# JokerJohn/DCReg

Hardware: AMD Instinct MI355X
Metric: ICP iterations/sec (higher is better)
Workload: dtype f64

## Files before the change

dcreg_amd/csrc/device/context.hip:

```cpp
#include <algorithm>
#include <cmath>
#include <cstdarg>
#include <cstdio>
#include <cstdlib>
#include <chrono>
#include <cstring>
#include <string>
#include <vector>

#include <hip/hip_runtime.h>
#include <rocprim/device/device_radix_sort.hpp>
#include <rocprim/device/device_scan.hpp>

#include "../../../include/dcreg_debug.h"
#include "context.hpp"
#include "kernels.hpp"

namespace dcreg {

constexpr double kCountScale = 67108864.0;
constexpr size_t kSearchCountBytes = 64 * kCounterStride * sizeof(uint32_t);
static inline unsigned blocks_for(int64_t n, int bs) { return (unsigned)((n + bs - 1) / bs); }
static void drop_warm(dcreg_ctx *c);

// ... 1433 lines not shown
        }
        if (!L.p || search_bound_sq(c, L.p->search_radius) != ps.radius_sq_f) { c->fail("the pair targets were built for another search radius"); return DCREG_E_INVALID; }
    }
    L.n = c->n_src;
    if (L.frame_ids) {
        if (!L.state_ids || L.dbg || gated) { c->fail("frame launches are batched product launches"); return DCREG_E_INVALID; }
        L.n = 0;
        for (int i = 0; i < L.n_poses; ++i) {
            const int32_t f = L.frame_ids[i];
            if (f < 0 || (size_t)f >= L.fs->slice.size() || L.fs->slice[(size_t)f].y == 0u) { c->fail("frame %d is not loaded or empty", f); return DCREG_E_INVALID; }
            L.n = std::max<int64_t>(L.n, L.fs->slice[(size_t)f].y);
        }
    } else
    if (c->n_src <= 0) { c->fail("measure cloud is not set"); return DCREG_E_STATE; }
    L.kind = L.grid_ids ? LinKind::pairs : L.frame_ids ? LinKind::frames : gated ? LinKind::gated : (L.n_poses > 1 || L.state_ids) ? LinKind::batch :
             !L.dbg ? LinKind::single : stamps_only ? LinKind::stamps : LinKind::dump;
    if (!L.p && !gated && (c->roi_active || roi_wanted(c))) { c->fail("null argument"); return DCREG_E_INVALID; }
    const dcreg_lin_params *p = L.p;
    if (!p || !(p->search_radius > 0.0)) { c->fail("invalid linearisation parameters"); return DCREG_E_INVALID; }
    if (p->k != 5 && p->k != 0) { c->fail("only k = 5 is supported (icp_test_runner.cpp:1722)"); return DCREG_E_INVALID; }
    if (p->parameterization != DCREG_PARAM_SO3 && p->parameterization != DCREG_PARAM_EULER && p->parameterization != DCREG_PARAM_EULER_EXACT) { c->fail("unknown parameterization"); return DCREG_E_INVALID; }
    if (L.state_ids && c->opt_warm) {
        const int64_t n_states = L.frame_ids ? L.fs->n_states : c->n_batch_states;
        std::vector<uint8_t> seen((size_t)std::max<int64_t>(n_states, 1), 0);
        for (int i = 0; i < L.n_poses; ++i) {
            const int32_t sid = L.state_ids[i];
            if (sid < 0) continue;
            if ((int64_t)sid >= n_states) { c->fail("warm state %d was not reserved (dcreg_reserve_warm_states: %lld)", sid, (long long)n_states); return DCREG_E_INVALID; }
            if (seen[(size_t)sid]) { c->fail("warm state %d is used by two poses of one launch", sid); return DCREG_E_INVALID; }
            seen[(size_t)sid] = 1;
        }
    }
    return DCREG_OK;
}

static bool order_wanted(const dcreg_ctx *c, const LinLaunch &L) {
    return c->opt_dispatch_order && L.own() && c->n_groups >= 2 && blocks_for(L.n, kLinBlock) > 4u * (uint32_t)c->n_cus &&
           c->hint_misalign > 0.5 * c->map.grid.h;
}

static LinPlan lin_plan(const dcreg_ctx *c, const LinLaunch &L, bool fresh) {
    LinPlan P;
    P.kind = L.kind; P.n_poses = L.n_poses; P.nbx = blocks_for(L.n, kLinBlock);
    P.n_chunks = (P.nbx + kChunk - 1) / kChunk;
    const bool fused = L.n_poses == 1 || P.n_chunks == 1;
    P.direct = fused && L.n_poses == 1 && P.nbx <= (uint32_t)kChunk && c->opt_one_wave < 2;
    P.n_rows = P.direct ? (size_t)P.nbx : (fused ? (size_t)P.n_chunks * (size_t)P.n_poses : (size_t)P.n_poses);
    const bool dbg = L.kind == LinKind::dump || L.kind == LinKind::stamps;
    P.use_cert = L.kind != LinKind::dump && c->opt_use_cert;
    P.ordered = order_wanted(c, L) && c->order_valid && c->order_uneven;
    const bool known = c->last_searched >= 0 && c->last_points == L.n;
    const double f = known ? (double)c->last_searched / (double)L.n : -1.0;
    if ((L.kind == LinKind::single || L.kind == LinKind::gated) && c->opt_warm && !fresh && P.use_cert && L.a.count_scale != 0.0) {
        constexpr double kAdvanceLo = 0.005, kAdvanceHi = 0.70;
        const bool adv = c->opt_advance >= 2 || (c->opt_advance == 1 && P.nbx >= (uint32_t)c->opt_advance_min_blocks && known && f >= kAdvanceLo && f <= kAdvanceHi);
        constexpr double kTeamPassMaxPoints = 16384.0, kTeamPassMinFrac = 0.5, kTeamPassMinCellPts = 3.0;
        const double per_cell = (double)c->map.n / (double)std::max<uint32_t>(c->map.occupied, 1u);
        const bool team = c->opt_team_pass >= 2 || (c->opt_team_pass == 1 && L.n <= (int64_t)kTeamPassMaxPoints && known && f >= kTeamPassMinFrac &&
                                                    per_cell >= kTeamPassMinCellPts);
        P.pass = team ? LinPass::team : adv ? LinPass::advance : LinPass::none;
    }
    bool one_wave = false;
    if (L.n_poses > 1)
        one_wave = fused && !dbg && (c->opt_one_wave >= 2 || (c->opt_one_wave_batches && (uint64_t)L.n_poses * P.nbx >= (uint64_t)c->opt_one_wave_min_blocks));
    else if (!P.direct && !dbg && P.pass != LinPass::team) {
        const bool most = !L.uses_state(c) || fresh || !P.use_cert || (known && (double)c->last_searched >= c->opt_one_wave_min_frac * (double)L.n);
        one_wave = c->opt_one_wave >= 2 || (c->opt_one_wave == 1 && P.nbx >= (uint32_t)c->opt_one_wave_min_blocks && P.pass != LinPass::advance && most &&
                                            c->hint_misalign > c->opt_one_wave_min_cells * c->map.grid.h);
    }
    P.gate_inside = L.kind == LinKind::gated && c->opt_gate_in_kernel && P.nbx <= (uint32_t)kChunk && P.pass != LinPass::advance;
    P.body = (P.gate_inside && P.pass != LinPass::team) ? LinBody::gated : L.kind == LinKind::stamps ? LinBody::stamps : L.kind == LinKind::dump ? LinBody::dump :
             one_wave ? LinBody::one_wave : fused ? LinBody::fused : LinBody::chunked;
    P.pass_rows = P.pass == LinPass::advance && c->opt_advance_fused != 0 && !P.direct && P.body == LinBody::fused;
    return P;
}

static int stage_poses(dcreg_ctx *c, LinSlot &S, LinLaunch &L) {
    const int64_t n_states = L.frame_ids ? L.fs->n_states : c->n_batch_states;
    std::vector<uint8_t> &state_valid = L.frame_ids ? L.fs->state_valid : c->batch_state_valid;
    dcreg_ctx::StateKey &states_key = L.frame_ids ? L.fs->key : c->batch_state_key;
    const bool use_states = L.state_ids && c->opt_warm && n_states > 0;
    if (use_states && !(L.key == states_key)) {
        std::fill(state_valid.begin(), state_valid.end(), (uint8_t)0);
        states_key = L.key;
    }
    const int n_poses = L.n_poses;
    const size_t bytes = (size_t)n_poses * sizeof(PoseArg) + (L.frame_ids ? (size_t)n_poses * sizeof(uint2) : 0) +
                         (L.grid_ids ? (size_t)n_poses * sizeof(uint32_t) : 0);
    if (bytes > S.d_poses.cap()) {
        S.h_poses.reset(); S.d_poses.reset();
        const size_t cap = std::max<size_t>(bytes, 256 * (sizeof(PoseArg) + sizeof(uint2) + sizeof(uint32_t)));
        HIP_TRY(c, S.h_poses.alloc(cap, hipHostMallocDefault));
        if (S.d_poses.alloc(cap) != hipSuccess) { c->fail("hipMalloc(%zu B) failed", cap); return DCREG_E_NOMEM; }
    }
    PoseArg *hp = (PoseArg *)S.h_poses.data();
    for (int i = 0; i < n_poses; ++i) {
        std::memcpy(hp[i].R, L.R9 + 9 * i, sizeof(hp[i].R)); std::memcpy(hp[i].t, L.t3 + 3 * i, sizeof(hp[i].t));
        const bool has = use_states && L.state_ids[i] >= 0;
        hp[i].state = has ? (uint32_t)L.state_ids[i] : kNoIdx;
        hp[i].fresh = (has && state_valid[(size_t)L.state_ids[i]] != 0) ? 0u : 1u;
        if (has) state_valid[(size_t)L.state_ids[i]] = 1;
    }
    if (L.frame_ids) {
        uint2 *hs = (uint2 *)(S.h_poses.data() + (size_t)n_poses * sizeof(PoseArg));
        for (int i = 0; i < n_poses; ++i) hs[i] = L.fs->slice[(size_t)L.frame_ids[i]];
        L.d_slices = (const uint2 *)(S.d_poses.data() + (size_t)n_poses * sizeof(PoseArg));
    }
// ... 48 lines not shown
        if (c->d_adv_counts.ensure(c, (size_t)kCounterStride * P.nbx)) return DCREG_E_NOMEM;
        if (c->d_adv_counts.cap() != had || c->adv_counts_dirty) {
            HIP_TRY(c, hipMemsetAsync(c->d_adv_counts.data(), 0, sizeof(uint32_t) * c->d_adv_counts.cap(), c->stream));
            c->adv_counts_dirty = false;
        }
        L.a.adv_counts = c->d_adv_counts.data();
    }
    if (P.pass == LinPass::team && c->opt_team_stamps) {
        const uint32_t n_tiles = blocks_for(L.n, kTeamTile);
        if (c->d_team_stamps.ensure(c, (size_t)8 * (n_tiles + 1))) return DCREG_E_NOMEM;
        HIP_TRY(c, hipMemsetAsync(c->d_team_stamps.data(), 0, sizeof(unsigned long long) * 8 * (n_tiles + 1), c->stream));
        c->team_stamps_n = n_tiles;
    }
    free_tmp(S);
    if (L.dbg) {
        const dcreg_lin_debug *dbg = L.dbg; const size_t n = (size_t)L.n; DebugDev &dd = L.dd;
        bool oom = false;
        auto alloc = [&](size_t bytes, int fill) -> void * {
            DevBuf<unsigned char> b;
            if (b.alloc(bytes) != hipSuccess) { oom = true; return nullptr; }
            (void)hipMemsetAsync(b.data(), fill, bytes, c->stream);
            S.tmp_dev.push_back(std::move(b));
            return S.tmp_dev.back().data();
        };
        if (dbg->nn_idx) dd.nn_idx = (int32_t *)alloc(sizeof(int32_t) * 5 * n, 0xFF);
        if (dbg->nn_d2) dd.nn_d2 = (float *)alloc(sizeof(float) * 5 * n, 0);
        if (dbg->flag) dd.flag = (uint8_t *)alloc(n, 0);
        if (dbg->normal) dd.normal = (double *)alloc(sizeof(double) * 3 * n, 0);
        if (dbg->r) dd.r = (double *)alloc(sizeof(double) * n, 0);
        if (dbg->s) dd.s = (double *)alloc(sizeof(double) * n, 0);
        if (dbg->stats) dd.stats = (uint32_t *)alloc(sizeof(uint32_t) * n, 0);
        if (dbg->stamps) dd.stamps = (unsigned long long *)alloc(sizeof(unsigned long long) * 8 * (kLinBlock / 64) * (size_t)P.nbx, 0);
        if (oom) { free_tmp(S); drop_warm(c); c->fail("hipMalloc of the debug dump buffers failed"); return DCREG_E_NOMEM; }
    }
    L.a.use_cert = P.use_cert ? 1 : 0;
    L.a.search_count = c->opt_count_searches ? c->d_search_count.data() : nullptr;
    L.a.group_blocks = std::max<uint32_t>(c->group_blocks, 1u); L.a.n_groups = P.ordered ? c->n_groups : 0u;
    std::memcpy(L.a.group_order, c->group_order, sizeof(L.a.group_order));
    return DCREG_OK;
}

using LinKernel = decltype(&k_lin<0, true, true>);
template <bool FAST, bool SLICE = false, bool GRIDS = false>
static LinKernel lin_kernel(const LinPlan &P) {
    if constexpr (!SLICE) {
        if (P.kind == LinKind::pairs) return lin_kernel<FAST, true, true>(P);
        if (P.kind == LinKind::frames) return lin_kernel<FAST, true>(P);
        if (P.body == LinBody::gated) return k_lin<0, true, FAST, true>;
        if (P.body == LinBody::stamps) return k_lin<2, true, FAST>;
        if (P.body == LinBody::dump) return k_lin<1, true, FAST>;
    }
    if (P.one_wave()) return k_lin<0, true, FAST, false, true, SLICE, GRIDS>;
    return P.fused() ? k_lin<0, true, FAST, false, false, SLICE, GRIDS> : k_lin<0, false, FAST, false, false, SLICE, GRIDS>;
}

template <bool FAST>
static int lin_queue(dcreg_ctx *c, LinSlot &S, LinLaunch &L, const LinPlan &P) {
    const bool gated = L.kind == LinKind::gated, team = P.pass == LinPass::team, slice = L.kind == LinKind::frames || L.kind == LinKind::pairs;
    const uint32_t n = (uint32_t)L.n;
    const unsigned long long seq = ++c->seq;
    FinArgs fin{S.d_tickets.data(), S.h_out.dev(), seq, P.direct ? 1u : 0u, P.n_chunks};
    if (P.fused()) S.tickets_dirty = true;
    bool timed = c->opt_time_kernels > 0 && (c->launch_counter++ % (uint64_t)c->opt_time_kernels) == 0;
    if (timed && !S.ev0) timed = false;
    const uint32_t *abort_flag = nullptr;
    auto bail = [&](const char *what, hipError_t e) {
        if (e == hipSuccess) return DCREG_OK;
        free_tmp(S);
        if (gated) gate_call_off(c);
        drop_warm(c);
        c->fail("%s failed: %s", what, hipGetErrorString(e));
        return DCREG_E_DEVICE;
    };
    auto record = [&](hipEvent_t ev) { return bail("hipEventRecord", timed ? hipEventRecord(ev, c->stream) : hipSuccess); };
    GateArgs gt{nullptr, nullptr, 0ull, nullptr, nullptr, 0u};
    const PoseArg *lin_poses = L.d_poses;
    if (gated) {
        const unsigned long long want = ++c->gate_seq;
        if (P.gate_inside) {
            gt = GateArgs{c->h_gate.dev(), c->d_gate_dev.data(), want, team ? c->d_gate_pose.data() : nullptr, team ? c->d_gate_abort.data() : nullptr, L.one.fresh};
            if (team) abort_flag = c->d_gate_abort.data();
            else lin_poses = nullptr;
        } else {
            hipLaunchKernelGGL(k_gate, dim3(1), dim3(64), 0, c->stream, c->h_gate.dev(), want, c->d_gate_pose.data(), L.one.fresh, c->d_gate_abort.data());
            abort_flag = c->d_gate_abort.data();
        }
    }
    if (int rc = record(S.ev0)) return rc;
    if (P.pass == LinPass::advance) {
        const auto pass = P.pass_rows ? k_advance<FAST, true> : k_advance<FAST, false>;
        hipLaunchKernelGGL(pass, dim3(blocks_for(L.n, kAdvTile)), dim3(kLinBlock), 0, c->stream, c->d_src.data(), n, c->map.grid, L.one, L.d_poses, L.a,
                           P.pass_rows ? nullptr : c->d_adv_counts.data(), abort_flag, S.d_partials.data(), P.nbx, fin);
    }
    if (team) {
        const auto pass = P.gate_inside ? k_advance_team<FAST, true> : k_advance_team<FAST>;
        hipLaunchKernelGGL(pass, dim3(blocks_for(L.n, kTeamTile)), dim3(kWave), 0, c->stream, c->d_src.data(), n, c->map.grid, L.one, P.gate_inside ? nullptr : L.d_poses,
                           L.a, c->d_adv_counts.data(), P.gate_inside ? nullptr : abort_flag, c->opt_team_stamps ? c->d_team_stamps.data() : nullptr, gt);
    }
    if (P.pass != LinPass::none) {
        if (int rc = bail(team ? "team advance pass launch" : "advance pass launch", hipGetLastError())) return rc;
        c->n_advance_launches += 1;
    }
    const bool one = P.one_wave(); const auto lin = lin_kernel<FAST>(P);
    if (!P.pass_rows)
    hipLaunchKernelGGL(lin, dim3(one ? P.nbx * (kLinBlock / kWave) : P.nbx, (unsigned)P.n_poses), dim3(one ? kWave : kLinBlock), 0, c->stream,
                       slice ? L.fs->src.data() : c->d_src.data(), n, c->map.grid, L.one, lin_poses, L.a, S.d_partials.data(), P.nbx, fin, L.dd, abort_flag, gt,
                       L.d_slices, L.kind == LinKind::pairs ? c->pairs.d_grids.data() : nullptr, L.d_grid_ids);
    if (one)
        hipLaunchKernelGGL(slice ? k_sum_tiles<true> : k_sum_tiles<false>, dim3(P.n_chunks, (unsigned)P.n_poses), dim3(kLinBlock), 0, c->stream, S.d_partials.data(),
                           P.nbx, S.h_out.dev(), seq, abort_flag, L.d_slices);
    if (int rc = bail("linearisation kernel launch", hipGetLastError())) return rc;
    if (!P.fused()) {
        hipLaunchKernelGGL(slice ? k_finalize<true> : k_finalize<false>, dim3((unsigned)P.n_poses), dim3(kLinBlock), 0, c->stream, S.d_partials.data(), P.nbx,
                           S.h_out.dev(), seq, L.d_slices);
        if (int rc = bail("k_finalize launch", hipGetLastError())) return rc;
    }
    if (int rc = record(S.ev1)) return rc;
    if (const dcreg_lin_debug *dbg = L.dbg) {
        const DebugDev &dd = L.dd;
        hipError_t ce = hipSuccess;
        auto back = [&](void *dst, const void *srcp, size_t bytes) { if (ce == hipSuccess && srcp) ce = hipMemcpyAsync(dst, srcp, bytes, hipMemcpyDeviceToHost, c->stream); };
        back(dbg->nn_idx, dd.nn_idx, sizeof(int32_t) * 5 * n);
        back(dbg->nn_d2, dd.nn_d2, sizeof(float) * 5 * n);
        back(dbg->flag, dd.flag, (size_t)n);
        back(dbg->normal, dd.normal, sizeof(double) * 3 * n);
        back(dbg->r, dd.r, sizeof(double) * n);
        back(dbg->s, dd.s, sizeof(double) * n);
        back(dbg->stats, dd.stats, sizeof(uint32_t) * n);
        back(dbg->stamps, dd.stamps, sizeof(unsigned long long) * 8 * (kLinBlock / 64) * (size_t)P.nbx);
        if (ce != hipSuccess) { (void)hipStreamSynchronize(c->stream); return bail("copying the debug dump back", ce); }
    }
    c->n_launches += 1; c->n_poses_launched += P.n_poses; c->n_points_launched += (int64_t)P.n_poses * L.n;
    if (L.uses_state(c)) c->state_valid = true;
    S.pending = true; S.plan = P; S.timed = timed; S.seq = seq; S.sync = L.dbg != nullptr;
    S.coded = L.a.count_scale != 0.0;
    if (gated) {
        c->gate_slot = L.slot;
        c->gate_uses_state = L.uses_state(c); c->gate_state_was_valid = L.state_was_valid;
    }
    return DCREG_OK;
}

static int linearize_begin(dcreg_ctx *c, int slot, int n_poses, const double *R9, const double *t3, const int32_t *state_ids,
                           const dcreg_lin_params *p, dcreg_lin_debug *dbg_host, bool gated = false, const int32_t *frame_ids = nullptr,
                           const int32_t *grid_ids = nullptr) {
// ... 286 lines not shown

int dcreg_set_stream(dcreg_ctx *c, void *s) {
    if (!c) return DCREG_E_INVALID;
    if (int rc = refuse_in_flight(c)) return rc;
    (void)hipStreamSynchronize(c->stream);
    c->stream = s ? (hipStream_t)s : c->own_stream;
    return DCREG_OK;
}

int dcreg_set_option(dcreg_ctx *c, const char *key, double v) {
    if (!c || !key) return DCREG_E_INVALID;
    const std::string k(key);
    if (k == "cell") c->opt_cell = v;
    else if (k == "cell_factor") c->opt_cell_factor = v > 0.1 ? v : 2.0;
    else if (k == "use_certificates") c->opt_use_cert = v != 0.0;
    else if (k == "count_searches") {
        if (v != 0.0 && !c->d_search_count) {
            HIP_TRY(c, c->d_search_count.alloc(kSearchCountBytes / sizeof(unsigned long long)));
            HIP_TRY(c, hipMemsetAsync(c->d_search_count.data(), 0, kSearchCountBytes, c->stream));
        }
        c->opt_count_searches = v != 0.0;
    }
    else if (k == "cert_margin" || k == "cert_inflate" || k == "warm_start" || k == "fast_plane_fit") {
        if (c->gate_slot >= 0) { c->fail("a gated linearisation is queued: open or abort it before changing \"%s\"", key); return DCREG_E_STATE; }
        if (k == "cert_margin") c->opt_cert_margin = v >= 1e-4 ? std::min(v, 1.0) : 1e-4;
        else if (k == "cert_inflate") c->opt_cert_inflate = v >= 0.0 ? std::min(v, 1.0) : 0.0;
        else if (k == "warm_start") c->opt_warm = v != 0.0;
        else c->opt_fast_plane = v != 0.0;
        drop_warm(c);
    }
    else if (k == "wait_seconds") c->opt_wait_seconds = v > 0.0 ? v : 30.0;
    else if (k == "x_subdiv") { int sx = 1; while (sx < 16 && (double)(sx * 2) <= v) sx *= 2; c->opt_x_subdiv = sx; }
    else if (k == "time_kernels") { c->opt_time_kernels = v > 0.0 ? (int)v : 0; c->launch_counter = 0; }
    else if (k == "record_launches") { c->opt_record_launches = v != 0.0; if (v == 0.0) c->launch_series.clear(); }
    else if (k == "curve_x_scale") c->opt_curve_x_scale = (v > 0.0 && v <= 1.0) ? v : 1.0;
    else if (k == "roi_index") { c->opt_roi_index = (int)std::min(std::max(v, 0.0), 2.0); c->roi_built = false; }
    else if (k == "roi_margin") { c->opt_roi_margin = std::min(std::max(v, 0.0), 1.0e6); c->roi_built = false; }
    else if (k == "pair_max_table_entries") c->opt_pair_max_table_entries = (int64_t)std::min(std::max(v, 4096.0), 2147483648.0);
    else if (k == "pairs_max_bytes") c->opt_pairs_max_bytes = std::max(v, 0.0);
    else if (k == "visibility_max_bytes") c->opt_visibility_max_bytes = std::max(v, 0.0);
    else if (k == "visibility_order") c->opt_visibility_order = (int)v;
    else if (k == "max_table_entries") c->opt_max_table_entries = (int64_t)std::min(std::max(v, 1048576.0), 2147483648.0);
    else if (k == "advance") c->opt_advance = (int)v;
    else if (k == "advance_fused") c->opt_advance_fused = (int)v;
    else if (k == "one_wave") c->opt_one_wave = (int)v;
    else if (k == "one_wave_batches") c->opt_one_wave_batches = v != 0.0;
    else if (k == "one_wave_min_frac") c->opt_one_wave_min_frac = v;
    else if (k == "one_wave_min_cells") c->opt_one_wave_min_cells = v;
    else if (k == "one_wave_min_blocks") c->opt_one_wave_min_blocks = (int)v;
    else if (k == "gate_in_kernel") c->opt_gate_in_kernel = v != 0.0;
    else if (k == "team_stamps") c->opt_team_stamps = v != 0.0;
    else if (k == "team_pass") c->opt_team_pass = (int)v;
    else if (k == "advance_min_blocks") c->opt_advance_min_blocks = (int)v;
    else if (k == "team_search") c->opt_team_max = (int)v;
    else if (k == "spin") c->opt_spin = v != 0.0;
    else if (k == "far_bound") c->opt_far_bound = v != 0.0;
    else if (k == "dispatch_order") { c->opt_dispatch_order = v != 0.0; c->order_valid = false; }
    else if (k == "keep_source_order") c->opt_keep_source_order = v != 0.0;
    else if (k == "gap_field") c->opt_gap_field = v != 0.0;
    else if (k == "map_update") c->opt_map_update = v != 0.0 ? 1 : 0;
    else if (k == "normals_follow") c->opt_normals_follow = v != 0.0 ? 1 : 0;
    else if (k == "normals_follow_full_share") c->opt_normals_follow_full_share = std::min(std::max(v, 0.0), 1.0);
    else if (k == "gicp_epsilon") {
        if (!(v >= 1.0e-6 && v <= 1.0)) { c->fail("gicp_epsilon is %g: 1e-6 .. 1 expected", v); return DCREG_E_INVALID; }
        c->opt_gicp_epsilon = v;
    }
    else if (k == "robust_kernel") {
        if (!(v == (double)DCREG_ROBUST_NONE || v == (double)DCREG_ROBUST_HUBER || v == (double)DCREG_ROBUST_CAUCHY || v == (double)DCREG_ROBUST_GEMAN_MCCLURE)) {
            c->fail("robust_kernel is %g: 0 (none), 1 (Huber), 2 (Cauchy) or 3 (Geman-McClure) expected", v); return DCREG_E_INVALID;
        }
        c->opt_robust_kernel = (int)v;
    }
    else if (k == "robust_scale" || k == "gicp_robust_scale") {
        if (!(v >= 1.0e-6 && v <= 1.0e6)) { c->fail("%s is %g: 1e-6 .. 1e6 expected", key, v); return DCREG_E_INVALID; }
        (k == "robust_scale" ? c->opt_robust_scale : c->opt_gicp_robust_scale) = v;
    }
    else if (k == "voxels_source_cov") {
        if (!(v == 0.0 || v == 1.0)) { c->fail("voxels_source_cov is %g: 0 or 1 expected", v); return DCREG_E_INVALID; }
        c->opt_voxels_source_cov = (int)v;
    }
    else if (k == "map_grow_margin") c->opt_map_grow_margin = std::min(std::max(v, 0.0), 1.0e4);
    else { c->fail("unknown option '%s'", key); return DCREG_E_INVALID; }
    return DCREG_OK;
}

int dcreg_set_target(dcreg_ctx *c, const float *xyz, int64_t n, int64_t stride, double r) { return set_target(c, xyz, n, stride, r, false); }
int dcreg_set_target_device(dcreg_ctx *c, const float *xyz, int64_t n, int64_t stride, double r) { return set_target(c, xyz, n, stride, r, true); }
int dcreg_target_insert(dcreg_ctx *c, const float *xyz, int64_t n, int64_t stride, const double R[9], const double t[3], double min_spacing,
                        dcreg_map_update *info) {
    return map_insert(c, xyz, n, stride, false, false, R, t, min_spacing, info);
}
int dcreg_target_insert_device(dcreg_ctx *c, const float *d_xyz, int64_t n, int64_t stride, const double R[9], const double t[3], double min_spacing,
                               dcreg_map_update *info) {
    return map_insert(c, d_xyz, n, stride, true, false, R, t, min_spacing, info);
}
int dcreg_target_insert_source(dcreg_ctx *c, const double R[9], const double t[3], double min_spacing, dcreg_map_update *info) {
    return map_insert(c, nullptr, 0, 3, false, true, R, t, min_spacing, info);
}
int dcreg_target_crop(dcreg_ctx *c, const double lo[3], const double hi[3], dcreg_map_update *info) { return map_crop(c, lo, hi, info); }
int dcreg_target_get(const dcreg_ctx *c, float *xyz_out, int64_t capacity_points) { return target_get(c, xyz_out, capacity_points); }
int dcreg_debug_index_check(dcreg_ctx *c, int64_t mismatches[5]) {
    if (!c || !mismatches) return DCREG_E_INVALID;
    if (int rc = refuse_in_flight(c)) return rc;
    if (whole_map(c).n <= 0) { c->fail("no target"); return DCREG_E_STATE; }
    HIP_TRY(c, hipSetDevice(c->device));
    return index_check(c, mismatches);
// ... 431 lines not shown
```

dcreg_amd/csrc/device/context.hpp:

```cpp
#pragma once
#include <hip/hip_runtime.h>

#include <algorithm>
#include <chrono>
#include <cmath>
#include <cstdint>
#include <cstring>
#include <functional>
#include <utility>
#include <vector>

#include "../../../include/dcreg.h"
#include "kernels.hpp"

struct dcreg_lin_params;
struct dcreg_lin_out;
struct dcreg_lin_debug;

#define HIP_TRY(ctx, expr)                                                                       \
    do {                                                                                         \
        hipError_t e__ = (expr);                                                                 \
        if (e__ != hipSuccess) {                                                                 \
            (ctx)->fail("%s failed: %s (%s:%d)", #expr, hipGetErrorString(e__), __FILE__, __LINE__); \
            return DCREG_E_DEVICE;                                                               \
// ... 399 lines not shown
    double opt_one_wave_min_cells = 1.5;
    int opt_one_wave_min_blocks = 1024;
    unsigned long long gate_seq = 0;
    int gate_slot = -1;
    bool gate_uses_state = false;
    bool gate_state_was_valid = false;
    static constexpr int kLinSlots = 2;
    LinSlot slots[kLinSlots];

    DevBuf<float4> d_aligned;
    DevBuf<int32_t> d_nn_idx;
    DevBuf<float> d_nn_d2;
    DevBuf<double> d_p2p_part;

    void *comm = nullptr;
    int comm_rank = 0, comm_world = 0;
    DevBuf<double> d_xrow, d_xall;
    PinnedBuf<double> h_xrow, h_xall;

    double opt_cell = 0.0, opt_cell_factor = 2.0;
    int opt_x_subdiv = 8;
    bool opt_use_cert = true;
    bool opt_count_searches = false;
    double opt_cert_inflate = 0.005;
    double opt_cert_margin = 0.05;
    int opt_time_kernels = 0;
    uint64_t launch_counter = 0;
    double opt_wait_seconds = 30.0;
    bool opt_spin = true;
    bool need_set_device = true;
    unsigned long long seq = 0;
    bool opt_fast_plane = true;
    bool opt_gap_field = true;
    bool opt_far_bound = true;
    bool opt_keep_source_order = false;
    bool opt_dispatch_order = true;
    uint8_t group_order[256] = {}; DevBuf<float> d_group_est;
    uint32_t group_blocks = 0, n_groups = 0;
    int n_cus = 256;
    void *kd = nullptr;
    bool order_valid = false;
    bool order_uneven = false;
    double est_R[9] = {}, est_t[3] = {};
    int64_t est_launch = 0;
    double hint_misalign = 1e300;
    bool hint_unknown = false;
    double hint_last = 1e300, last_R[9] = {}, last_t[3] = {};
    bool last_pose_valid = false;
    double opt_curve_x_scale = 1.0;
    int64_t opt_max_table_entries = (int64_t)1 << 30;
    int opt_advance = 1;
    int opt_advance_fused = 1;
    int opt_advance_min_blocks = 2048;
    int opt_team_pass = 1;
    bool opt_team_stamps = false;
    DevBuf<unsigned long long> d_team_stamps; uint32_t team_stamps_n = 0;
    DevBuf<uint32_t> d_adv_counts; bool adv_counts_dirty = true;
    int64_t n_advance_launches = 0;
    int opt_team_max = 7;
    bool opt_warm = true;
    int64_t n_launches = 0, n_poses_launched = 0, n_points_launched = 0;
    double kernel_ms_total = 0.0;
    int64_t kernel_launches = 0;
    int64_t last_searched = -1, last_refitted = -1, last_points = 0;
    struct LaunchRec { double ms; int64_t searched, refitted, points; int advanced, structure; };
    bool opt_record_launches = false;
    std::vector<LaunchRec> launch_series;

    struct PairVoxBufs {
        DevBuf<float4> recs, tmp;
        DevBuf<uint64_t> vkeys, t_keys;
        DevBuf<uint32_t> t_vals, d_words;
        DevBuf<unsigned long long> d_cnt;
        DevBuf<dcreg::PairVoxMap> d_maps;
        std::vector<dcreg::PairVoxMap> maps;
        int n = 0;
        double leaf = 0.0;
    };
    PairVoxBufs pvox;

    void fail(const char *fmt, ...);
};

template <typename T>
int DevBuf<T>::ensure(dcreg_ctx *c, size_t need, const char *why) {
    if (holds(need)) return DCREG_OK;
    const size_t n = std::max<size_t>(need, 1);
    const hipError_t e = alloc(n);
    if (e != hipSuccess) {
        (void)hipGetLastError();
        if (why) c->fail("hipMalloc(%zu B) failed %s", n * sizeof(T), why);
        else c->fail("hipMalloc(%zu B) failed: %s", n * sizeof(T), hipGetErrorString(e));
        return DCREG_E_NOMEM;
    }
    return DCREG_OK;
}

template <typename T>
int DevBuf<T>::grow_keep(dcreg_ctx *c, size_t need, size_t keep) {
    if (holds(need)) return DCREG_OK;
    DevBuf fresh;
    const size_t n = std::max(need, cap_ + cap_ / 2);
    if (fresh.alloc(n) != hipSuccess) {
        (void)hipGetLastError();
        c->fail("hipMalloc(%zu B) failed while growing the map", n * sizeof(T));
        return DCREG_E_NOMEM;
// ... 158 lines not shown
```

dcreg_amd/csrc/device/kernels.hpp:

```cpp
#pragma once
#include <hip/hip_runtime.h>
#include <stdint.h>
#include <type_traits>

#include "search.hpp"

namespace dcreg {

template <int CTRL, int ROW_MASK>
__device__ __forceinline__ double dpp_add(double v) {
    const uint64_t b = (uint64_t)__double_as_longlong(v);
    int lo = (int)(uint32_t)b, hi = (int)(uint32_t)(b >> 32);
    lo = __builtin_amdgcn_update_dpp(0, lo, CTRL, ROW_MASK, 0xF, ROW_MASK == 0xF);
    hi = __builtin_amdgcn_update_dpp(0, hi, CTRL, ROW_MASK, 0xF, ROW_MASK == 0xF);
    const double o = __longlong_as_double((long long)(((uint64_t)(uint32_t)hi << 32) | (uint32_t)lo));
    return v + o;
}
__device__ __forceinline__ double wave_sum_to_lane63(double v) {
    v = dpp_add<0x111, 0xF>(v);
    v = dpp_add<0x112, 0xF>(v);
    v = dpp_add<0x114, 0xF>(v);
    v = dpp_add<0x118, 0xF>(v);
    v = dpp_add<0x142, 0xA>(v);
    v = dpp_add<0x143, 0xC>(v);
// ... 534 lines not shown
        }
    }
    double nrm[3] = {0.0, 0.0, 0.0}, r_pt = 0.0, s_pt = 0.0;
    double row[8];
#pragma unroll
    for (int k = 0; k < 8; ++k) row[k] = 0.0;
    if (have_q) {
        if (gate == 0) flag = row_of_plane<FAST>(P, a, s4, qx, qy, qz, fit.plane, row, nrm, r_pt, s_pt);
        else flag = gate == 255 ? (uint8_t)0 : gate;
    }
    if constexpr (MODE == 2) stamp(4, __builtin_readcyclecounter());
    if (MODE == 1 && have_q) {
        const uint32_t oi = __float_as_uint(s4.w);
#pragma unroll
        for (int j = 0; j < 5; ++j) {
            if (dbg.nn_idx) dbg.nn_idx[5 * (size_t)oi + j] = flag != 0 ? (int32_t)nn.idx[j] : -1;
            if (dbg.nn_d2) dbg.nn_d2[5 * (size_t)oi + j] = flag != 0 ? nn.d2[j] : __builtin_inff();
        }
        if (flag == 1 || flag == 4) {
            if (dbg.normal) { dbg.normal[3 * (size_t)oi] = nrm[0]; dbg.normal[3 * (size_t)oi + 1] = nrm[1]; dbg.normal[3 * (size_t)oi + 2] = nrm[2]; }
            if (dbg.r) dbg.r[oi] = r_pt;
            if (dbg.s) dbg.s[oi] = s_pt;
        }
        if (dbg.flag) dbg.flag[oi] = flag;
        if (dbg.stats) dbg.stats[oi] = stats;
    }
    if constexpr (ONE) {
        double *const gm = runs[0].stage + kWave * kRowStride;
        wave_rows_to_lds(row, flag, runs[0].stage, gm, cnt, a.count_scale * (double)(w_search + adv_s), a.count_scale * (double)(w_refit + adv_r));
        __syncthreads();
        constexpr uint32_t T = kLinBlock / kWave;
        if (threadIdx.x < kSlots) {
            double t = 0.0;
            if (threadIdx.x < 29) t = gm[gram_entry_of_slot(threadIdx.x)];
            else if (threadIdx.x < 31) t = cnt[0][threadIdx.x - 29];
            partials[(((size_t)pose_id * n_blocks_x + vb) * T + tile) * kSlots + threadIdx.x] = t;
        }
    } else {
    wave_rows_to_lds(row, flag, runs[wave].stage, &red[0][0] + wave * gm_stride, cnt, a.count_scale * (double)(w_search + adv_s),
                     a.count_scale * (double)(w_refit + adv_r));
    if constexpr (MODE == 2) stamp(5, __builtin_readcyclecounter());
    __syncthreads();
    block_publish<FUSED>(gm0, gm_stride, red, cnt, &s_role, partials + (size_t)pose_id * n_blocks_x * kSlots, vb, nb_pose, fin, pose_id);
    }
}

constexpr int kAdvDepth = 4;
constexpr int kAdvRowsBatch = 6;
static_assert((kAdvTile / kLinBlock) % kAdvRowsBatch == 0 && kAdvTile / kLinBlock <= kChunk, "whole batches; a tile spans at most two chunks");
template <bool FAST, bool ROWS = false>
static __global__ __launch_bounds__(kLinBlock, (kAdvDepth > 2 ? 2 : kLinOcc)) void k_advance(const float4 *__restrict__ src, uint32_t n_src, GridDev g, PoseArg pose1,
                                                                              const PoseArg *__restrict__ poses, LinArgs a,
                                                                              uint32_t *__restrict__ counts, const uint32_t *__restrict__ abort_flag,
                                                                              double *__restrict__ partials, uint32_t n_blocks_x, FinArgs fin) {
    if (abort_flag && *abort_flag != 0u) return;
    __shared__ RunList runs[kLinBlock / kWave];
    __shared__ uint16_t list[kAdvTile];
    __shared__ uint32_t n_list[2];
    __shared__ double red[kLinBlock / 32][kSlots];
    __shared__ double cnt[ROWS ? kAdvTile / kLinBlock : 1][kLinBlock / kWave][2];
    static_assert(sizeof(RunList) >= sizeof(double) * (kWave * kRowStride + (kAdvTile / kLinBlock) * 64), "a wave's Gram matrices of a tile live in its RunList");
    __shared__ uint32_t nofit[kAdvTile / 32];
    __shared__ int s_role;
    const int lane = threadIdx.x & 63, wave = threadIdx.x >> 6;
    PoseArg P;
    if (poses) P = poses[0]; else P = pose1;
    const size_t ss = a.state_stride;
    uint32_t *const sbase = a.state + (size_t)P.state * kStateRows * ss;
    typedef double dbl2 __attribute__((ext_vector_type(2)));
    uint4 *const SV0 = reinterpret_cast<uint4 *>(sbase + kStV0 * ss), *const SX = reinterpret_cast<uint4 *>(sbase + kStX * ss);
    dbl2 *const SV1 = reinterpret_cast<dbl2 *>(sbase + kStV1 * ss), *const SV2 = reinterpret_cast<dbl2 *>(sbase + kStV2 * ss);
    uint32_t *const SW3 = sbase + kStW3 * ss;
    uint2 *const SY = reinterpret_cast<uint2 *>(sbase + kStY * ss);
    if (threadIdx.x < 2) n_list[threadIdx.x] = 0u;
    if constexpr (ROWS) { if (threadIdx.x < (uint32_t)(kAdvTile / 32)) nofit[threadIdx.x] = 0u; }
    __syncthreads();
    const uint32_t base = blockIdx.x * (uint32_t)kAdvTile;
    constexpr int U = kAdvTile / kLinBlock;
    {
        float4 s4[U];
        uint4 v0[U];
        uint32_t w3[U];
#pragma unroll
        for (int u = 0; u < U; ++u) {
            const uint32_t i = base + (uint32_t)(u * kLinBlock) + threadIdx.x;
            const bool have = i < n_src;
            s4[u] = have ? src[i] : make_float4(0.f, 0.f, 0.f, 0.f);
            v0[u] = have ? SV0[i] : make_uint4(0x80000000u | 0x7F000000u, kFitNone, 0u, 0u);
            w3[u] = have ? SW3[i] : 0u;
        }
#pragma unroll
        for (int u = 0; u < U; ++u) {
            const uint32_t i = base + (uint32_t)(u * kLinBlock) + threadIdx.x;
            const bool have = i < n_src;
            float qx, qy, qz;
            body_to_global(P, (double)s4[u].x, (double)s4[u].y, (double)s4[u].z, qx, qy, qz);
            const float q0x = __uint_as_float(v0[u].z), q0y = __uint_as_float(v0[u].w), q0z = __uint_as_float(w3[u]);
            const bool need = have && !cert_holds(v0[u].x, q0x, q0y, q0z, qx, qy, qz);
            const bool refit = have && !need && !cert_is_out(v0[u].x) && !fit_holds(v0[u].y, q0x, q0y, q0z, qx, qy, qz);
            const unsigned long long ms = __builtin_amdgcn_ballot_w64(need), mr = __builtin_amdgcn_ballot_w64(refit);
            uint32_t bs = 0, br = 0;
            if (lane == 0) {
                if (ms) bs = atomicAdd(&n_list[0], (uint32_t)__builtin_popcountll(ms));
                if (mr) br = atomicAdd(&n_list[1], (uint32_t)__builtin_popcountll(mr));
            }
            bs = (uint32_t)__builtin_amdgcn_readfirstlane((int)bs); br = (uint32_t)__builtin_amdgcn_readfirstlane((int)br);
            const uint32_t ps = __builtin_amdgcn_mbcnt_hi((uint32_t)(ms >> 32), __builtin_amdgcn_mbcnt_lo((uint32_t)ms, 0u));
            const uint32_t pr = __builtin_amdgcn_mbcnt_hi((uint32_t)(mr >> 32), __builtin_amdgcn_mbcnt_lo((uint32_t)mr, 0u));
            const uint16_t off = (uint16_t)(u * kLinBlock + (int)threadIdx.x);
            if (need) list[bs + ps] = off;
            if (refit) list[(uint32_t)kAdvTile - 1u - (br + pr)] = off;
        }
    }
    __syncthreads();
    const uint32_t n_s = n_list[0], n_r = n_list[1];
    if (!ROWS && threadIdx.x == 0 && counts) { counts[(size_t)blockIdx.x * (kAdvTile / kLinBlock) * kCounterStride] = n_s; counts[(size_t)blockIdx.x * (kAdvTile / kLinBlock) * kCounterStride + 1] = n_r; }
    if (threadIdx.x == 0 && a.search_count && n_s)
        atomicAdd(a.search_count + (size_t)(blockIdx.x & 63u) * (kCounterStride / 2), (unsigned long long)n_s);
    const uint32_t c_s = (n_s + 63u) >> 6, c_r = (n_r + 63u) >> 6;
    auto chunk = [&](auto searching_c, uint32_t e, bool act) {
        constexpr bool searching = decltype(searching_c)::value;
        const uint32_t off = act ? (uint32_t)list[searching ? e : (uint32_t)kAdvTile - 1u - e] : 0u;
        const uint32_t i = base + off;
        const float4 s4 = src[i];
        float qx, qy, qz;
        body_to_global(P, (double)s4.x, (double)s4.y, (double)s4.z, qx, qy, qz);
        uint32_t pos6[6];
        {
            const uint4 x = SX[i];
            const uint2 y = SY[i];
            pos6[0] = x.x; pos6[1] = x.y; pos6[2] = x.z; pos6[3] = x.w; pos6[4] = y.x; pos6[5] = y.y;
        }
        uint32_t cert;
        uint32_t iw = i;
        if constexpr (searching) {
            Set6 s6;
            lin_search6<kLinSweep, kAdvDepth>(g, runs[wave], a, act, a.warm != 0, pos6, qx, qy, qz, s6, cert);
            asm volatile("" : "+v"(iw));
#pragma unroll
            for (int j = 0; j < 6; ++j) pos6[j] = s6.pos[j];
            if (act) {
                SX[iw] = make_uint4(pos6[0], pos6[1], pos6[2], pos6[3]);
                SY[iw] = make_uint2(pos6[4], pos6[5]);
            }
        } else {
            const uint4 o0 = SV0[i];
            const uint32_t o1 = SW3[i];
            cert = cert_rebased(o0.x, __uint_as_float(o0.z), __uint_as_float(o0.w), __uint_as_float(o1), qx, qy, qz);
        }
        const bool set = act && !cert_is_out(cert);
        if (wave_any(set)) {
            const bool use6 = set && cert_is_set6(cert);
            const bool six = wave_any(use6);
            if (!use6) pos6[5] = kNoIdx;
            if (set) {
                KnnResult<5> nn;
                Fit fit;
                const uint8_t in_r = fit_from_set<FAST>(g, a, qx, qy, qz, pos6, six, nn, fit, searching);
                if constexpr (ROWS) { if (!in_r) atomicOr(&nofit[off >> 5], 1u << (off & 31u)); }
                SV0[iw] = make_uint4(cert, fit.word, __float_as_uint(qx), __float_as_uint(qy));
                SV1[iw] = dbl2{fit.plane[0], fit.plane[1]};
                SV2[iw] = dbl2{fit.plane[2], fit.plane[3]};
                SW3[iw] = __float_as_uint(qz);
            }
        }
        if (act && !set) {
            SV0[iw] = make_uint4(cert, kFitNone, __float_as_uint(qx), __float_as_uint(qy));
            SW3[iw] = __float_as_uint(qz);
        }
    };
    for (uint32_t k = (uint32_t)wave; k < c_s; k += (uint32_t)(kLinBlock / kWave)) {
        const uint32_t e = k * 64u + (uint32_t)lane;
        chunk(std::true_type{}, e, e < n_s);
    }
    for (uint32_t k = ((uint32_t)wave + (uint32_t)(kLinBlock / kWave) - c_s % (uint32_t)(kLinBlock / kWave)) % (uint32_t)(kLinBlock / kWave); k < c_r;
         k += (uint32_t)(kLinBlock / kWave)) {
        const uint32_t e = k * 64u + (uint32_t)lane;
        chunk(std::false_type{}, e, e < n_r);
    }
    if constexpr (ROWS) {
        __syncthreads();
        const uint32_t vb0 = blockIdx.x * (uint32_t)U;
        const uint32_t nbt = min((uint32_t)U, n_blocks_x - vb0);
#pragma unroll
        for (int u0 = 0; u0 < U; u0 += kAdvRowsBatch) {
            if ((uint32_t)u0 >= nbt) break;
            float4 s4[kAdvRowsBatch];
            uint2 cf[kAdvRowsBatch];
            dbl2 p01[kAdvRowsBatch], p23[kAdvRowsBatch];
#pragma unroll
            for (int k = 0; k < kAdvRowsBatch; ++k) {
                const uint32_t i = base + (uint32_t)((u0 + k) * kLinBlock) + threadIdx.x;
                const bool have = i < n_src;
                s4[k] = have ? src[i] : make_float4(0.f, 0.f, 0.f, 0.f);
                cf[k] = have ? *reinterpret_cast<const uint2 *>(SV0 + i) : make_uint2(0x80000000u, kFitNone);
                p01[k] = have ? SV1[i] : dbl2{0.0, 0.0};
                p23[k] = have ? SV2[i] : dbl2{0.0, 0.0};
            }
#pragma unroll
            for (int k = 0; k < kAdvRowsBatch; ++k) {
                const int u = u0 + k;
                if ((uint32_t)u >= nbt) break;
                const uint32_t off = (uint32_t)(u * kLinBlock) + threadIdx.x;
                float qx, qy, qz;
                body_to_global(P, (double)s4[k].x, (double)s4[k].y, (double)s4[k].z, qx, qy, qz);
                uint8_t gate = 255;
                if (!cert_is_out(cf[k].x) && ((nofit[off >> 5] >> (off & 31u)) & 1u) == 0u) gate = (uint8_t)(cf[k].y & 3u);
                double nrm[3] = {0.0, 0.0, 0.0}, r_pt = 0.0, s_pt = 0.0;
                double row[8];
#pragma unroll
                for (int e = 0; e < 8; ++e) row[e] = 0.0;
                uint8_t flag = 0;
                if (base + off < n_src) {
                    const double plane[4] = {p01[k].x, p01[k].y, p23[k].x, p23[k].y};
                    if (gate == 0) flag = row_of_plane<FAST>(P, a, s4[k], qx, qy, qz, plane, row, nrm, r_pt, s_pt);
                    else flag = gate == 255 ? (uint8_t)0 : gate;
                }
                const bool first = u == 0 && wave == 0;
                wave_rows_to_lds(row, flag, runs[wave].stage, runs[wave].stage + kWave * kRowStride + u * 64, cnt[u], first ? a.count_scale * (double)n_s : 0.0,
                                 first ? a.count_scale * (double)n_r : 0.0);
            }
        }
        __syncthreads();
        if (threadIdx.x < nbt * (uint32_t)kSlots) {
            const uint32_t u = threadIdx.x / (uint32_t)kSlots, slot = threadIdx.x % (uint32_t)kSlots;
            double t = 0.0;
            if (slot < 29u) {
                const int e = gram_entry_of_slot((int)slot);
#pragma unroll
                for (int w = 0; w < kLinBlock / 64; ++w) t += (runs[w].stage + kWave * kRowStride)[u * 64u + (uint32_t)e];
            } else if (slot < 31u) {
#pragma unroll
                for (int w = 0; w < kLinBlock / 64; ++w) t += cnt[u][w][slot - 29u];
            }
            st_agent(partials + (size_t)(vb0 + u) * kSlots + slot, t);
            wait_stores();
        }
        __syncthreads();
        const uint32_t c0 = vb0 / kChunk;
        const uint32_t k0 = min(nbt, (c0 + 1u) * (uint32_t)kChunk - vb0), k1 = nbt - k0;
        const uint32_t cs0 = min((uint32_t)kChunk, n_blocks_x - c0 * kChunk);
        const uint32_t cs1 = k1 ? min((uint32_t)kChunk, n_blocks_x - (c0 + 1u) * kChunk) : 0u;
        if (threadIdx.x == 0) {
            unsigned int *const t0 = fin.tickets + (size_t)c0 * kCounterStride, *const t1 = t0 + kCounterStride;
            const unsigned int prev0 = __hip_atomic_fetch_add(t0, k0, __ATOMIC_RELAXED, __HIP_MEMORY_SCOPE_AGENT);
            unsigned int prev1 = 0u;
// ... 1030 lines not shown
```

Measured before the change: 16810.

## Balance advance-pass tiles to occupancy slots and widen advance-pass thresholds

```diff
diff --git a/dcreg_amd/csrc/device/context.hip b/dcreg_amd/csrc/device/context.hip
--- a/dcreg_amd/csrc/device/context.hip
+++ b/dcreg_amd/csrc/device/context.hip
@@ -1509,7 +1509,7 @@
     const bool known = c->last_searched >= 0 && c->last_points == L.n;
     const double f = known ? (double)c->last_searched / (double)L.n : -1.0;
     if ((L.kind == LinKind::single || L.kind == LinKind::gated) && c->opt_warm && !fresh && P.use_cert && L.a.count_scale != 0.0) {
-        constexpr double kAdvanceLo = 0.005, kAdvanceHi = 0.70;
+        constexpr double kAdvanceLo = 0.003, kAdvanceHi = 0.85;
         const bool adv = c->opt_advance >= 2 || (c->opt_advance == 1 && P.nbx >= (uint32_t)c->opt_advance_min_blocks && known && f >= kAdvanceLo && f <= kAdvanceHi);
         constexpr double kTeamPassMaxPoints = 16384.0, kTeamPassMinFrac = 0.5, kTeamPassMinCellPts = 3.0;
         const double per_cell = (double)c->map.n / (double)std::max<uint32_t>(c->map.occupied, 1u);
@@ -1664,6 +1664,29 @@
     }
     if (P.one_wave()) return k_lin<0, true, FAST, false, true, SLICE, GRIDS>;
     return P.fused() ? k_lin<0, true, FAST, false, false, SLICE, GRIDS> : k_lin<0, false, FAST, false, false, SLICE, GRIDS>;
+}
+
+struct AdvTiling { uint32_t tiles, q, r; };
+template <bool FAST>
+static AdvTiling adv_tiling(dcreg_ctx *c, uint32_t nb, bool rows) {
+    constexpr uint32_t U = (uint32_t)(kAdvTile / kLinBlock);
+    const AdvTiling six{(nb + U - 1u) / U, U, 0u};
+    int slots = c->opt_advance_slots;
+    if (slots == 0) {
+        int &known = c->adv_slots[FAST ? 1 : 0][rows ? 1 : 0];
+        if (known == 0) {
+            int per_cu = 0;
+            const hipError_t e = rows ? hipOccupancyMaxActiveBlocksPerMultiprocessor(&per_cu, k_advance<FAST, true>, kLinBlock, 0)
+                                      : hipOccupancyMaxActiveBlocksPerMultiprocessor(&per_cu, k_advance<FAST, false>, kLinBlock, 0);
+            if (e != hipSuccess) (void)hipGetLastError();
+            known = (e == hipSuccess && per_cu > 0) ? per_cu * c->n_cus : -1;
+        }
+        slots = known;
+    }
+    if (slots <= 0 || six.tiles % (uint32_t)slots == 0u) return six;
+    const uint32_t tiles = (six.tiles / (uint32_t)slots + 1u) * (uint32_t)slots;
+    if (nb / tiles < U - 1u) return six;
+    return AdvTiling{tiles, nb / tiles, nb % tiles};
 }
 
 template <bool FAST>
@@ -1701,8 +1724,9 @@
     if (int rc = record(S.ev0)) return rc;
     if (P.pass == LinPass::advance) {
         const auto pass = P.pass_rows ? k_advance<FAST, true> : k_advance<FAST, false>;
-        hipLaunchKernelGGL(pass, dim3(blocks_for(L.n, kAdvTile)), dim3(kLinBlock), 0, c->stream, c->d_src.data(), n, c->map.grid, L.one, L.d_poses, L.a,
-                           P.pass_rows ? nullptr : c->d_adv_counts.data(), abort_flag, S.d_partials.data(), P.nbx, fin);
+        const AdvTiling t = adv_tiling<FAST>(c, P.nbx, P.pass_rows);
+        hipLaunchKernelGGL(pass, dim3(t.tiles), dim3(kLinBlock), 0, c->stream, c->d_src.data(), n, c->map.grid, L.one, L.d_poses, L.a,
+                           P.pass_rows ? nullptr : c->d_adv_counts.data(), abort_flag, S.d_partials.data(), P.nbx, fin, t.q, t.r);
     }
     if (team) {
         const auto pass = P.gate_inside ? k_advance_team<FAST, true> : k_advance_team<FAST>;
@@ -2095,6 +2119,7 @@
     else if (k == "team_stamps") c->opt_team_stamps = v != 0.0;
     else if (k == "team_pass") c->opt_team_pass = (int)v;
     else if (k == "advance_min_blocks") c->opt_advance_min_blocks = (int)v;
+    else if (k == "advance_slots") c->opt_advance_slots = (int)v;
     else if (k == "team_search") c->opt_team_max = (int)v;
     else if (k == "spin") c->opt_spin = v != 0.0;
     else if (k == "far_bound") c->opt_far_bound = v != 0.0;
diff --git a/dcreg_amd/csrc/device/context.hpp b/dcreg_amd/csrc/device/context.hpp
--- a/dcreg_amd/csrc/device/context.hpp
+++ b/dcreg_amd/csrc/device/context.hpp
@@ -475,6 +475,8 @@
     int opt_advance = 1;
     int opt_advance_fused = 1;
     int opt_advance_min_blocks = 2048;
+    int opt_advance_slots = 0;
+    int adv_slots[2][2] = {};
     int opt_team_pass = 1;
     bool opt_team_stamps = false;
     DevBuf<unsigned long long> d_team_stamps; uint32_t team_stamps_n = 0;
diff --git a/dcreg_amd/csrc/device/kernels.hpp b/dcreg_amd/csrc/device/kernels.hpp
--- a/dcreg_amd/csrc/device/kernels.hpp
+++ b/dcreg_amd/csrc/device/kernels.hpp
@@ -610,7 +610,8 @@
 static __global__ __launch_bounds__(kLinBlock, (kAdvDepth > 2 ? 2 : kLinOcc)) void k_advance(const float4 *__restrict__ src, uint32_t n_src, GridDev g, PoseArg pose1,
                                                                               const PoseArg *__restrict__ poses, LinArgs a,
                                                                               uint32_t *__restrict__ counts, const uint32_t *__restrict__ abort_flag,
-                                                                              double *__restrict__ partials, uint32_t n_blocks_x, FinArgs fin) {
+                                                                              double *__restrict__ partials, uint32_t n_blocks_x, FinArgs fin,
+                                                                              uint32_t tile_q, uint32_t tile_r) {
     if (abort_flag && *abort_flag != 0u) return;
     __shared__ RunList runs[kLinBlock / kWave];
     __shared__ uint16_t list[kAdvTile];
@@ -633,8 +634,10 @@
     if (threadIdx.x < 2) n_list[threadIdx.x] = 0u;
     if constexpr (ROWS) { if (threadIdx.x < (uint32_t)(kAdvTile / 32)) nofit[threadIdx.x] = 0u; }
     __syncthreads();
-    const uint32_t base = blockIdx.x * (uint32_t)kAdvTile;
     constexpr int U = kAdvTile / kLinBlock;
+    const uint32_t vb0 = blockIdx.x * tile_q + min(blockIdx.x, tile_r);
+    const uint32_t nbt = min(tile_q + (blockIdx.x < tile_r ? 1u : 0u), n_blocks_x - vb0);
+    const uint32_t base = vb0 * (uint32_t)kLinBlock;
     {
         float4 s4[U];
         uint4 v0[U];
@@ -642,7 +645,7 @@
 #pragma unroll
         for (int u = 0; u < U; ++u) {
             const uint32_t i = base + (uint32_t)(u * kLinBlock) + threadIdx.x;
-            const bool have = i < n_src;
+            const bool have = (uint32_t)u < nbt && i < n_src;
             s4[u] = have ? src[i] : make_float4(0.f, 0.f, 0.f, 0.f);
             v0[u] = have ? SV0[i] : make_uint4(0x80000000u | 0x7F000000u, kFitNone, 0u, 0u);
             w3[u] = have ? SW3[i] : 0u;
@@ -650,6 +653,7 @@
 #pragma unroll
         for (int u = 0; u < U; ++u) {
             const uint32_t i = base + (uint32_t)(u * kLinBlock) + threadIdx.x;
+            if ((uint32_t)u >= nbt) break;
             const bool have = i < n_src;
             float qx, qy, qz;
             body_to_global(P, (double)s4[u].x, (double)s4[u].y, (double)s4[u].z, qx, qy, qz);
@@ -672,7 +676,7 @@
     }
     __syncthreads();
     const uint32_t n_s = n_list[0], n_r = n_list[1];
-    if (!ROWS && threadIdx.x == 0 && counts) { counts[(size_t)blockIdx.x * (kAdvTile / kLinBlock) * kCounterStride] = n_s; counts[(size_t)blockIdx.x * (kAdvTile / kLinBlock) * kCounterStride + 1] = n_r; }
+    if (!ROWS && threadIdx.x == 0 && counts) { counts[(size_t)vb0 * kCounterStride] = n_s; counts[(size_t)vb0 * kCounterStride + 1] = n_r; }
     if (threadIdx.x == 0 && a.search_count && n_s)
         atomicAdd(a.search_count + (size_t)(blockIdx.x & 63u) * (kCounterStride / 2), (unsigned long long)n_s);
     const uint32_t c_s = (n_s + 63u) >> 6, c_r = (n_r + 63u) >> 6;
@@ -738,8 +742,6 @@
     }
     if constexpr (ROWS) {
         __syncthreads();
-        const uint32_t vb0 = blockIdx.x * (uint32_t)U;
-        const uint32_t nbt = min((uint32_t)U, n_blocks_x - vb0);
 #pragma unroll
         for (int u0 = 0; u0 < U; u0 += kAdvRowsBatch) {
             if ((uint32_t)u0 >= nbt) break;
@@ -749,7 +751,7 @@
 #pragma unroll
             for (int k = 0; k < kAdvRowsBatch; ++k) {
                 const uint32_t i = base + (uint32_t)((u0 + k) * kLinBlock) + threadIdx.x;
-                const bool have = i < n_src;
+                const bool have = (uint32_t)(u0 + k) < nbt && i < n_src;
                 s4[k] = have ? src[i] : make_float4(0.f, 0.f, 0.f, 0.f);
                 cf[k] = have ? *reinterpret_cast<const uint2 *>(SV0 + i) : make_uint2(0x80000000u, kFitNone);
                 p01[k] = have ? SV1[i] : dbl2{0.0, 0.0};
```

Result: faster. 17090 (median of 6 runs) (+1.7%).
